# Ladme/groan_rs

Hardware: AMD Instinct MI355X
Metric: frames/sec RMSD-fit, 1e6 atoms triclinic, 1/2/4/8 GPUs; HBM GB/s vs peak (higher is better)
Workload: dtype f32 (fp64 accumulators)

## Files before the change

### groan_rs_amd/csrc/gr_api.hip

```cpp
#include <hip/hip_runtime.h>

#include <cmath>
#include <cstdio>
#include <cstdlib>
#include <cstring>
#include <map>
#include <string>
#include <vector>

#include "../../include/groan_hip.h"
#include "gr_batch.h"
#include "gr_container.h"
#include "gr_kernels.h"
#include "gr_hot.h"
#include "gr_resident.h"
#include "gr_small.h"
#include "gr_xtc.h"
#include "gr_shape.h"
#include "gr_xtc_dev.h"
#include "gr_xtc_enc_dev.h"
#include "gr_trr.h"
#include "gr_cellgrid.h"
#include "gr_textio.h"
#include "gr_pool.h"
// ... 499 lines not shown
        if ((spins & 1023u) == 1023u && std::chrono::steady_clock::now() - t0 > std::chrono::milliseconds(20)) {
            c->small_sync_fallbacks++;
            HIPCHK(c, hipStreamSynchronize(c->stream));
            if (w[0] != seq || w[words - 1] != seq) return fail(c, GR_E_HIP, "a single-wave kernel ended without publishing its result");
            break;
        }
    }
    std::atomic_thread_fence(std::memory_order_acquire);
    c->small_calls++;
    return GR_OK;
}

static int res_next_epoch(gr_ctx *c, uint32_t *epoch) {
    if (++c->res_epoch == 0u) {
        HIPCHK(c, hipStreamSynchronize(c->stream));
        if (c->res_wgrec) HIPCHK(c, hipMemset(c->res_wgrec, 0, c->res_wgrec_cap * sizeof(unsigned long long)));
        HIPCHK(c, hipMemset(c->res_rec, 0, (size_t)GR_MAX_BATCH * 16 * sizeof(unsigned long long)));
        HIPCHK(c, hipMemset(c->res_abort + 2, 0, 2 * sizeof(uint32_t)));
        c->res_epoch = 1u;
    }
    *epoch = c->res_epoch;
    return GR_OK;
}
static int res_test_no_start(gr_ctx *c, uint32_t epoch) {
    if (!c->res_test_no_start) return GR_OK;
    const unsigned long long two = 2ull | ((unsigned long long)epoch << 32);
    c->res_test_no_start = 0;
    HIPCHK(c, hipMemcpyAsync(c->res_abort + 2, &two, sizeof two, hipMemcpyHostToDevice, c->stream));
    HIPCHK(c, hipStreamSynchronize(c->stream));
    return GR_OK;
}
template <int MODE>
static int res_close(gr_ctx *c, uint32_t nb, const double *fit_partials, uint32_t nparts, double sum_w, uint32_t epoch, bool fresh, uint32_t *seq) {
    const uint32_t sq = c->res_seq + 1u;
    k_res_close<MODE><<<dim3(nb), dim3(64), 0, c->stream>>>(fit_partials, nparts, sum_w, c->state_dev, c->res_rec, epoch, fresh ? 1u : 0u, c->res_abort, c->res_closed + nb,
                                                        c->res_out_dev->st, c->res_out_dev->words, &c->res_out_dev->seq, sq);
    HIPCHK(c, hipGetLastError());
    c->res_seq = sq; c->res_closed += nb; *seq = sq;
    return GR_OK;
}
static int res_collect(gr_ctx *c, uint32_t seq, uint32_t nb, uint32_t epoch, bool *started) {
    volatile uint32_t *w = &c->res_out->seq;
    const auto t0 = std::chrono::steady_clock::now();
    for (uint32_t spins = 0; *w != seq; ++spins) {
        if ((spins & 1023u) == 1023u && std::chrono::steady_clock::now() - t0 > std::chrono::milliseconds(20)) {
            c->res_sync_fallbacks++;
            HIPCHK(c, hipStreamSynchronize(c->stream));
            if (*w != seq) return fail(c, GR_E_HIP, "the kernel behind the resident pass ended without publishing its results");
            break;
        }
    }
    std::atomic_thread_fence(std::memory_order_acquire);
    memcpy(c->state_host, c->res_out->st, (size_t)nb * sizeof(GrFrameState));
    memcpy(c->res_words_host, c->res_out->words, 12 * sizeof(uint32_t));
    for (int k = 0; k < 2; ++k) { const uint32_t v = c->res_words_host[8 + k]; c->res_words_host[8 + k] = v - c->res_late_seen[k]; c->res_late_seen[k] = v; }
    *started = c->res_words_host[2] == 1u && c->res_words_host[3] == epoch;
    if (!*started || c->res_words_host[0]) HIPCHK(c, hipStreamSynchronize(c->stream));
    return GR_OK;
}

int center_stage(gr_ctx *c, uint32_t first_slot, uint32_t nf, const GrSel &sel, int kind, int weighted,
                 int mass_first, int target, int only_status = 0) {
    if (small_ok(c, sel)) {
        k_center_small_stage<<<dim3(nf), dim3(64), 0, c->stream>>>(c->frames, c->frame_stride, first_slot, c->masses, sel, c->boxes_dev, kind, weighted, mass_first, target, c->state_dev, only_status);
        HIPCHK(c, hipGetLastError());
        return GR_OK;
    }
    uint32_t nch = chunks_for(sel);
    if (nf > 1 && nch >= 8) nch &= ~7u;
    const dim3 grid(nch, nf), wg(GR_WG);
    if (kind == 0) k_center_sums<0><<<grid, wg, 0, c->stream>>>(c->frames, c->frame_stride, first_slot, c->masses, sel, c->boxes_dev, c->state_dev, weighted, c->cen_partials, only_status);
    else if (kind == 1) k_center_sums<1><<<grid, wg, 0, c->stream>>>(c->frames, c->frame_stride, first_slot, c->masses, sel, c->boxes_dev, c->state_dev, weighted, c->cen_partials, only_status);
    else k_center_sums<2><<<grid, wg, 0, c->stream>>>(c->frames, c->frame_stride, first_slot, c->masses, sel, c->boxes_dev, c->state_dev, weighted, c->cen_partials, only_status);
    k_center_finalize<<<dim3(nf), dim3(GR_WG), 0, c->stream>>>(c->cen_partials, nch, c->boxes_dev, first_slot, kind, weighted, mass_first, target, sel.n, c->state_dev, only_status);
    HIPCHK(c, hipGetLastError());
    return GR_OK;
}

int pbc_center_stages(gr_ctx *c, uint32_t first_slot, uint32_t nf, const GrSel &sel, int weighted, int only_status = 0) {
    if (small_ok(c, sel) && only_status == 0) {
        k_center_small_pbc<<<dim3(nf), dim3(64), 0, c->stream>>>(c->frames, c->frame_stride, first_slot, c->masses, sel, c->boxes_dev, weighted, c->state_dev);
        HIPCHK(c, hipGetLastError());
        return GR_OK;
    }
    int st = center_stage(c, first_slot, nf, sel, 1, 0, 0, 0, only_status);
    if (st != GR_OK) return st;
    return center_stage(c, first_slot, nf, sel, 2, weighted, 0, 1, only_status);
}

// ... 972 lines not shown

static int states_from_prechecks(gr_ctx *c, const grb::PreView &pre) {
    if (pre.all_ok) return state_reset(c, pre.n);
    for (uint32_t f = 0; f < pre.n; ++f) { GrFrameState z = {}; z.err_index = GR_NOIDX; z.status = pre.pre[f]; c->state_host[f] = z; }
    HIPCHK(c, hipMemcpyAsync(c->state_dev, c->state_host, pre.n * sizeof(GrFrameState), hipMemcpyHostToDevice, c->stream));
    return GR_OK;
}
int gr_group_center_batch(gr_ctx *c, uint32_t first_slot, uint32_t n_frames, const char *group, int kind, int weighted, float *out, int *status_out) try {
    int st = slot_check(c, first_slot, n_frames); if (st) return st;
    (void)hipSetDevice(c->device);
    const Group *g = need_group(c, group, st, true); if (!g) return st;
    if (kind != GR_CENTER_NAIVE && kind != GR_CENTER_ESTIMATE && kind != GR_CENTER_PBC) return fail(c, GR_E_INVALID_ARG, "unknown centre kind");
    const GrSel sel = make_sel(*g);
    grb::FirstError<gr_ctx> fe;
    for (const auto [b0, nb, s0] : grb::Segments{ first_slot, n_frames }) {
        const grb::Prechecks pre(c, { b0, nb, s0 }, box_checks(c, kind != GR_CENTER_NAIVE));
        SlotUse use(c, s0, nb);
        st = states_from_prechecks(c, pre); if (st) return st;
        if (kind == GR_CENTER_NAIVE) st = center_stage(c, s0, nb, sel, 0, weighted, 0, 1);
        else if (kind == GR_CENTER_ESTIMATE) st = center_stage(c, s0, nb, sel, 1, weighted, 1, 1);
        else st = center_onepass_ok(c, sel) ? pbc_center_onepass(c, s0, nb, sel, weighted) : pbc_center_stages(c, s0, nb, sel, weighted);
        if (st) return st;
        st = fetch_states(c, nb); if (st) return st;
        std::vector<GrFrameState> res;
        st = center_redo_fallbacks(c, s0, nb, sel, weighted, res); if (st) return st;
        for (uint32_t f = 0; f < nb; ++f) {
            const int s = grb::close_frame(c, fe, pre, f, status_out, [&] { return frame_status(c, res[f]); });
            if (out) for (int k = 0; k < 3; ++k) out[3 * (size_t)(b0 + f) + k] = (s == GR_OK) ? res[f].com[k] : NAN;
        }
    }
    return fe.finish(c);
} catch (...) { return gr_abi_guard(); }
static int center_resident(gr_ctx *c, uint32_t s0, uint32_t nb, const GrSel &all, const GrSel &csel, int dim_mask, int weighted,
                           const std::vector<int> &pre, bool fresh_states, std::vector<uint8_t> &done, std::vector<uint8_t> &torn, bool &ran) {
    done.assign(nb, 0); torn.assign(nb, 0); ran = false;
    if (!c->center_resident || !csel.contiguous || csel.masked || !all.contiguous || all.start != 0 || all.n != c->n) return GR_OK;
    {
        bool ortho = true;
        for (uint32_t f = 0; f < nb; ++f) if (pre[f] == GR_OK) { ortho = c->boxes_host[s0 + f].ortho != 0; break; }
        if (c->resident == 1 && (uint64_t)csel.n * 100 < c->n * (ortho ? 15u : 3u)) return GR_OK;
    }
    if (small_ok(c, csel)) return GR_OK;
    uint32_t streams = 1, gwg = GR_RES_GROUPS;
    const uint32_t wgs = resident_wgs(c, true, nb, all, &streams, &gwg);
    if (!wgs) return GR_OK;
    if (!resident_acquire(c->device)) return GR_OK;
    struct Release { gr_ctx *c; ~Release() { resident_release(c->device); } } release{ c };
    hipStream_t S = c->stream;
    const uint32_t res_stream = wgs * streams;
    const uint32_t n_fin = std::min<uint32_t>(streams > 8 ? GR_RES_MAX_FIN : 8, c->res_max_wgs - res_stream);
    const size_t rec_words = (size_t)nb * ((wgs + GR_RES_REC_PAD - 1u) & ~(uint32_t)(GR_RES_REC_PAD - 1u)) * GR_RES_REC_WORDS;
    if (rec_words > c->res_wgrec_cap) {
        if (c->res_wgrec) (void)hipFree(c->res_wgrec);
        c->res_wgrec = nullptr; c->res_wgrec_cap = 0;
        HIPCHK(c, hipMalloc(&c->res_wgrec, rec_words * sizeof(unsigned long long)));
        HIPCHK(c, hipMemsetAsync(c->res_wgrec, 0, rec_words * sizeof(unsigned long long), S));
        c->res_wgrec_cap = rec_words;
    }
    GrResCtl ctl;
    memset(&ctl, 0, sizeof ctl);
    { const int se = res_next_epoch(c, &ctl.epoch); if (se) return se; }
    ctl.wgrec = c->res_wgrec; ctl.rec = c->res_rec; ctl.abort = c->res_abort; ctl.progress = c->res_progress; ctl.n_stream = res_stream; ctl.n_fin = n_fin;
    ctl.checkin_target = c->res_checkin + res_stream + n_fin; ctl.fresh_states = fresh_states ? 1u : 0u;
    ctl.wgs_frame = wgs; ctl.streams = streams; ctl.groups_wg = gwg;
    ctl.team_waves = resident_team_waves(wgs, streams);
    ctl.patience_ticks = (unsigned long long)c->wall_khz * 3000ull; ctl.start_ticks = (unsigned long long)c->wall_khz * 200ull;
    ctl.test_abort_frame = c->res_test_abort_at; c->res_test_abort_at = 0xFFFFFFFFu;
    ctl.metro_t16 = c->res_metro_ns >= 100 ? (uint32_t)std::min<uint64_t>(0xFFFFFFFFull, (uint64_t)c->res_metro_ns * (uint64_t)c->wall_khz * 16ull / 1000000ull) : 0u;
    ctl.metro_lead = (uint32_t)((uint64_t)c->wall_khz * 2000ull / 1000000ull);
    ctl.cen_weighted = weighted ? 1u : 0u; ctl.cen_dim_mask = (uint32_t)dim_mask;
    float *frames = c->frames; size_t stride = c->frame_stride; uint32_t slot0 = s0, nfr = nb, natoms = (uint32_t)c->n;
    const float *masses = c->masses; GrSel sel_arg = csel; const GrBox *boxes = c->boxes_dev; GrPlanDev plan; memset(&plan, 0, sizeof plan);
    GrFrameState *states = c->state_dev; double *fparts = nullptr;
    void *args[] = { &frames, &stride, &slot0, &nfr, &natoms, &masses, &sel_arg, &boxes, &plan, &states, &fparts, &ctl };
    bool ubox = true;
    for (uint32_t f = 1; f < nb && ubox; ++f) ubox = memcmp(&c->boxes_host[s0 + f], &c->boxes_host[s0], sizeof(GrBox)) == 0;
    const bool fit_last = c->res_fit_last ? c->res_fit_last == 2 : (uint64_t)res_stream * 10u >= (uint64_t)c->res_max_wgs * 9u;
    { const int sn = res_test_no_start(c, ctl.epoch); if (sn) return sn; }
    if (hipLaunchKernel(resident_center_fn(ubox, fit_last), dim3(res_stream + n_fin), dim3(GrResShape::LANES), args, GrResShape::LDS_BYTES, S) != hipSuccess) {
        (void)hipGetLastError();
        c->res_max_wgs = 0;
        return GR_OK;
    }
    c->res_checkin += res_stream + n_fin;
    uint32_t seq = 0; bool started = false;
    { const int sc = res_close<1>(c, nb, nullptr, 0u, 1.0, ctl.epoch, fresh_states, &seq); if (sc) return sc; }
    { const int sc = res_collect(c, seq, nb, ctl.epoch, &started); if (sc) return sc; }
    c->res_last_streams = streams;
    if (!started) {
        c->res_handshake_misses++;
        c->res_backoff = c->res_backoff ? std::min<uint32_t>(c->res_backoff * 2u, 1024u) : 4u;
        c->res_skip = c->res_backoff;
        return GR_OK;
    }
    c->res_backoff = 0;
    c->cen_res_launches++;
    if (fresh_states) c->res_lean_segments++;
    ran = true;
#ifdef GR_EXP_STEPTIME
    if (getenv("GR_STEPTIME")) {
        unsigned long long st[32];
        if (hipMemcpy(st, c->res_abort + 16, sizeof st, hipMemcpyDeviceToHost) == hipSuccess) {
            const double turns_ = (double)((nb + streams - 1) / streams + GrResShape::K);
            const char *who[4] = { "wg 0 wave 0", "wg 0 wave 5", "wg mid wave 0", "wg mid wave 5" };
            for (int w = 0; w < 4; ++w) {
                fprintf(stderr, "center steptime %-14s ticks/turn:", who[w]);
                double tot = 0; for (int k = 0; k < 7; ++k) tot += (double)st[w * 8 + k];
                const char *nm[7] = { "gate", "request", "rows+sums", "reduce+handover", "record wait", "fit+stores", "park" };
                for (int k = 0; k < 7; ++k) fprintf(stderr, " %s %.0f", nm[k], (double)st[w * 8 + k] / turns_);
// ... 39 lines not shown
        k_translate_wrap_rows<<<dim3(tiles * 3u, nb), dim3(64), 0, c->stream>>>(c->frames + (size_t)s0 * c->frame_stride, c->frame_stride, sel, c->boxes_dev + s0, c->state_dev, mode, dim_mask,
                                                                            v ? v[0] : 0.f, v ? v[1] : 0.f, v ? v[2] : 0.f, c->bad_dev);
        HIPCHK(c, hipGetLastError());
    } else if (g->n) {
        const uint64_t units = sel.contiguous ? ((uint64_t)sel.n + 3) / 4 + 128 : (sel.masked & 2u) ? ((uint64_t)sel.span + 3) / 4 + 128 : sel.n;
        const uint32_t nwg = (uint32_t)std::min<uint64_t>((units + GR_WG - 1) / GR_WG, 4096);
        k_translate_wrap<<<dim3(nwg, nb), dim3(GR_WG), stream_lds(c, GR_STREAM_WGS_CU_DEFAULT), c->stream>>>(c->frames + (size_t)s0 * c->frame_stride, c->frame_stride, sel, c->boxes_dev + s0, c->state_dev, mode, dim_mask,
                                                                       v ? v[0] : 0.f, v ? v[1] : 0.f, v ? v[2] : 0.f, c->bad_dev);
        HIPCHK(c, hipGetLastError());
    }
    HIPCHK(c, hipMemcpyAsync(c->bad_host, c->bad_dev, 4 * (size_t)nb * sizeof(uint32_t), hipMemcpyDeviceToHost, c->stream));
    HIPCHK(c, hipMemcpyAsync(c->state_host, c->state_dev, nb * sizeof(GrFrameState), hipMemcpyDeviceToHost, c->stream));
    HIPCHK(c, hipStreamSynchronize(c->stream));
    for (uint32_t f = 0; f < nb; ++f)
        grb::close_frame(c, fe, pre, f, status_out, [&]() -> int {
            if (mode == 1 && c->state_host[f].status != GR_OK) return frame_status(c, c->state_host[f]);
            return c->bad_host[4 * f] != GR_NOIDX ? fail(c, GR_E_NO_POSITION, "atom has no position", c->bad_host[4 * f]) : (int)GR_OK;
        });
    return GR_OK;
}
static int translate_batch_api(gr_ctx *c, uint32_t first_slot, uint32_t n_frames, const char *group, const float *v, const char *center_group, int dim, int weighted, int *status_out) {
    int st = slot_check(c, first_slot, n_frames); if (st) return st;
    (void)hipSetDevice(c->device);
    const Group *g = find_group(c, group ? group : "all");
    if (!g) return fail(c, GR_E_GROUP_NOT_FOUND, group);
    const Group *cg = nullptr;
    if (center_group) {
        cg = need_group(c, center_group, st, true); if (!cg) return st;
        if (dim < 0 || dim > 7) return fail(c, GR_E_INVALID_ARG, "bad dimension");
    }
    static const int mask[8] = { 0, 1, 2, 4, 3, 5, 6, 7 };
    grb::FirstError<gr_ctx> fe;
    for (const auto [b0, nb, s0] : grb::Segments{ first_slot, n_frames }) {
        const grb::Prechecks pre(c, { b0, nb, s0 }, box_checks(c, true));
        SlotUse use(c, s0, nb);
        const bool states_unset = cg != nullptr && pre.all_ok;
        if (!states_unset) { st = states_from_prechecks(c, pre); if (st) return st; }
        std::vector<uint8_t> done(nb, 0), torn(nb, 0);
        bool ran = false;
        if (cg) { st = center_resident(c, s0, nb, make_sel(*g), make_sel(*cg), mask[dim], weighted, pre.codes, states_unset, done, torn, ran); if (st) return st; }
        bool any_done = false;
        for (uint32_t f = 0; f < nb; ++f) any_done = any_done || done[f];
        if (any_done) {
            for (uint32_t f = 0; f < nb; ++f) {
                if (!done[f]) continue;
                grb::close_frame(c, fe, pre, f, status_out, [&]() -> int {
                    if (torn[f]) return fail(c, GR_E_HIP, "the resident atoms_center pass stalled while this frame was being moved: some of its atoms carry the new coordinates, others the original ones (frame index in gr_last_error_index)", pre.b0 + f);
                    return frame_status(c, c->state_host[f]);
                });
            }
            for (uint32_t a = 0; a < nb; ) {
                if (done[a]) { ++a; continue; }
                uint32_t b = a;
                while (b < nb && !done[b]) ++b;
                const grb::PreView run = pre.sub(a, b);
                st = states_from_prechecks(c, run); if (st) return st;
                st = center_stage(c, s0 + a, b - a, make_sel(*cg), 1, weighted, 1, 0); if (st) return st;
                st = translate_batch(c, run, g, v, 1, mask[dim], status_out, fe); if (st) return st;
                a = b;
            }
            continue;
        }
        if (ran || states_unset) { st = states_from_prechecks(c, pre); if (st) return st; }
        if (cg) { st = center_stage(c, s0, nb, make_sel(*cg), 1, weighted, 1, 0); if (st) return st; }
        st = translate_batch(c, pre, g, v, cg ? 1 : 2, cg ? mask[dim] : 7, status_out, fe); if (st) return st;
    }
    return fe.finish(c);
}
int gr_group_translate_batch(gr_ctx *c, uint32_t first_slot, uint32_t n_frames, const char *group, const float v[3], int *status_out) try {
    if (!c) return GR_E_INVALID_ARG;
    if (!v) return fail(c, GR_E_INVALID_ARG, "vector is NULL");
    return translate_batch_api(c, first_slot, n_frames, group, v, nullptr, 7, 0, status_out);
} catch (...) { return gr_abi_guard(); }
// ... 125 lines not shown
    case GR_TUNE_RESIDENT_FIT_LAST: if (value < 0 || value > 2) break; c->res_fit_last = (int)value; return GR_OK;
    case GR_TUNE_STREAM_WGS_PER_CU: if (value < 0 || value > 8) break; c->stream_wgs_cu = (int)value; return GR_OK;
    case GR_TUNE_CENTER_RESIDENT: if (value < 0 || value > 1) break; c->center_resident = (int)value; return GR_OK;
    case GR_TUNE_TRANSLATE_ROWS: if (value < 0 || value > 1) break; c->translate_rows = (int)value; return GR_OK;
    case GR_TUNE_RESIDENT_FILL: if (value < 1 || value > 16) break; c->res_fill16 = (int)value; return GR_OK;
    case GR_TUNE_RESIDENT_GROUPS: if (value != 2) break; return GR_OK;
    case GR_TUNE_TEST_RESIDENT_NO_START: c->res_test_no_start = value ? 1 : 0; return GR_OK;
    case GR_TUNE_TEST_RESIDENT_ABORT_AT: c->res_test_abort_at = value < 0 ? 0xFFFFFFFFu : (uint32_t)value; return GR_OK;
    default: break;
    }
    return fail(c, GR_E_INVALID_ARG, "unknown tuning key or value out of range");
} catch (...) { return gr_abi_guard(); }

static int rmsd_exact(gr_rmsd_plan *p, gr_ctx *c, const GrSel &sel, uint32_t first_slot, uint32_t nf, int fit) {
    int st = pbc_center_stages(c, first_slot, nf, sel, 1); if (st) return st;
    if (small_ok(c, sel)) {
        k_rmsd_small<1><<<dim3(nf), dim3(64), 0, c->stream>>>(c->frames, c->frame_stride, first_slot, c->masses, sel, c->boxes_dev, p->dev, c->state_dev, 1, nullptr, nullptr, 0u);
    } else {
        const uint32_t nch = chunks_for(sel);
        k_rmsd_accum<1><<<dim3(nch, nf), dim3(GR_WG), 0, c->stream>>>(c->frames, c->frame_stride, first_slot, c->masses, sel, c->boxes_dev, p->dev, c->state_dev, c->acc_partials);
        k_rmsd_finalize<1><<<dim3(nf), dim3(GR_WG), 0, c->stream>>>(c->acc_partials, nch, c->frames, c->frame_stride, first_slot, sel, c->boxes_dev, p->dev, c->state_dev);
    }
    if (fit) {
        const uint32_t gx = (uint32_t)std::min<uint64_t>(((c->n >> 2) + GR_WG * 4 - 1) / (GR_WG * 4) + 1, 1024);
        k_fit_pk<false><<<dim3(gx, nf), dim3(GR_WG), 0, c->stream>>>(c->frames, c->frame_stride, first_slot, (uint32_t)c->n, c->boxes_dev, p->dev, c->state_dev, c->masses, sel, nullptr);
    }
    HIPCHK(c, hipGetLastError());
    return GR_OK;
}

static int segment_begin(gr_rmsd_plan *p, uint32_t s0, uint32_t nb, int fit) {
    gr_ctx *c = p->target;
    Pending &q = p->pend;
    q = Pending();
    q.s0 = s0; q.nb = nb; q.fit = fit; q.active = true;
    SlotUse use(c, s0, nb);
    const Group *g = find_group(c, p->group.c_str());
    q.pre.assign(nb, GR_OK); q.pre_idx.assign(nb, 0); q.pre_msg.assign(nb, std::string());
    for (uint32_t f = 0; f < nb; ++f) {
        int s = box_check(c, s0 + f);
        if (s == GR_OK && !g) s = fail(c, GR_E_GROUP_NOT_FOUND, p->group);
        if (s == GR_OK && g->n == 0) s = fail(c, GR_E_EMPTY_GROUP, p->group);
        q.pre[f] = s;
        if (s != GR_OK) { q.pre_msg[f] = c->err; q.pre_idx[f] = c->err_index; }
        q.any_ok = q.any_ok || s == GR_OK;
    }
    if (!q.any_ok) return GR_OK;
    const GrSel sel = make_sel(*g);
    q.sel = sel; q.group_n = g->n; q.has_group = true;
    if (!p->resolved || p->resolved_epoch != c->epoch) {
        p->resolved_epoch = c->epoch;
        bool same = (g->n == p->n_ref);
        if (same) { size_t k = 0; for (uint64_t i : grc::expand(g->blocks)) { const float a = c->masses_host[i], b = p->w_host[k++]; if (!(a == b)) { same = false; break; } } }
        p->dev.w_is_mass = same ? 1u : 0u; p->resolved = true;
        p->span_ok = p->p_span_dev != nullptr && g->masked && g->mask_dev != nullptr && g->blocks == p->ref_blocks;
    }
    q.consistent = (g->n == p->n_ref);
    const bool fast_asked = c->two_pass && c->rmsd_fast && p->dev.w_is_mass != 0 && g->n >= c->rmsd_fast_min && ((!fit && sel.contiguous) || (sel.masked && p->span_ok));
    const bool small = q.consistent && !p->exact && small_ok(c, sel) && !fast_asked;
    if (small && nb == 1) {
        q.small = true; q.small_seq = ++c->small_seq;
        k_rmsd_small<0><<<dim3(1), dim3(64), 0, c->stream>>>(c->frames, c->frame_stride, s0, c->masses, sel, c->boxes_dev, p->dev,
                                                         c->state_dev, 0, c->small_state_dev, c->small_flag_dev, q.small_seq);
        if (fit) k_fit_pk<false><<<dim3(fit_grid(c, 1), 1), dim3(GR_WG), 0, c->stream>>>(c->frames, c->frame_stride, s0, (uint32_t)c->n, c->boxes_dev, p->dev, c->state_dev, c->masses, sel, nullptr);
        p->fit_behind_small = fit != 0;
        HIPCHK(c, hipGetLastError());
        return GR_OK;
    }
    bool states_unset = false;
    {
        bool all_ok = true;
        for (uint32_t f = 0; f < nb; ++f) all_ok = all_ok && q.pre[f] == GR_OK;
        states_unset = all_ok;
        if (!all_ok) {
            for (uint32_t f = 0; f < nb; ++f) { GrFrameState z = {}; z.err_index = GR_NOIDX; z.status = q.pre[f]; c->state_host[f] = z; }
            HIPCHK(c, hipMemcpyAsync(c->state_dev, c->state_host, nb * sizeof(GrFrameState), hipMemcpyHostToDevice, c->stream));
        }
    }
    auto zero_states = [&]() -> int { if (!states_unset) return GR_OK; states_unset = false; return state_reset(c, nb); };
    int st;
    if (!(q.consistent && !p->exact && !small)) { st = zero_states(); if (st) return st; }
    if (small) {
        k_rmsd_small<0><<<dim3(nb), dim3(64), 0, c->stream>>>(c->frames, c->frame_stride, s0, c->masses, sel, c->boxes_dev, p->dev, c->state_dev, 1, nullptr, nullptr, 0u);
        if (fit) k_fit_pk<false><<<dim3(fit_grid(c, nb), nb), dim3(GR_WG), 0, c->stream>>>(c->frames, c->frame_stride, s0, (uint32_t)c->n, c->boxes_dev, p->dev, c->state_dev, c->masses, sel, nullptr);
        HIPCHK(c, hipGetLastError());
    } else if (!q.consistent) {
        st = pbc_center_stages(c, s0, nb, sel, 1); if (st) return st;
    } else if (p->exact) {
        st = rmsd_exact(p, c, sel, s0, nb, fit); if (st) return st;
    } else {
        const uint32_t sb = c->sub_batch;
        const bool lite = fit && sel.contiguous && c->two_pass;
        const bool msk = sel.masked && p->span_ok;
        const bool fast = c->two_pass && c->rmsd_fast && p->dev.w_is_mass != 0 && g->n >= c->rmsd_fast_min && ((!fit && sel.contiguous) || msk);
        q.rmsd_fast = fast;
        p->dev.fast_sigmas = (float)c->rmsd_fast_sigmas;
        GrPlanDev plan_span = p->dev; plan_span.p = p->p_span_dev;
        const uint32_t n_groups = (nb + sb - 1) / sb;
        if (lite) {
            size_t need = 0;
            for (uint32_t f0 = 0; f0 < nb; f0 += sb) need = std::max(need, (size_t)nb * fit_grid(c, std::min<uint32_t>(sb, nb - f0)) * (GR_WG / 64));
            if (need > c->fit_partials_cap) {
                if (c->fit_partials) (void)hipFree(c->fit_partials);
                c->fit_partials = nullptr; c->fit_partials_cap = 0;
                HIPCHK(c, hipMalloc(&c->fit_partials, need * sizeof(double)));
// ... 40 lines not shown
                if (c->res_metro_ns >= 100) period_ns = (uint32_t)c->res_metro_ns;
                else if (c->res_metro_ns == 0) {
                    gr_ctx::Metro &m = c->metro;
                    if (m.shape != shape) { m = gr_ctx::Metro(); m.shape = shape; }
                    if (m.off_for) m.off_for--;
                    else if (m.free_ns > 0) period_ns = (uint32_t)(m.T_ns + 0.5);
                    q.res_metro_auto = true;
                }
                q.res_metro_ns = period_ns;
                ctl.metro_t16 = (uint32_t)std::min<uint64_t>(0xFFFFFFFFull, (uint64_t)period_ns * (uint64_t)c->wall_khz * 16ull / 1000000ull);
                ctl.metro_lead = (uint32_t)((uint64_t)c->wall_khz * 2000ull / 1000000ull);
            }
#ifdef GR_EXP_STEPTIME
            {
                static unsigned long long *dbg_dev = nullptr;
                if (!dbg_dev) (void)hipMalloc(&dbg_dev, (size_t)GR_MAX_CHUNKS * 8 * 4 * sizeof(unsigned long long));
                ctl.dbg = getenv("GR_STEPTIME") ? dbg_dev : nullptr;
                g_steptime_dbg = ctl.dbg;
            }
#endif
#ifdef GR_EXP_TIMELINE
            {
                static unsigned long long *tl_dev = nullptr; static size_t tl_cap = 0;
                if (nb > tl_cap) { if (tl_dev) (void)hipFree(tl_dev); tl_dev = nullptr; tl_cap = 0; if (hipMalloc(&tl_dev, (size_t)nb * 8 * sizeof(unsigned long long)) == hipSuccess) tl_cap = nb; }
                ctl.tl = getenv("GR_TIMELINE") ? tl_dev : nullptr;
                if (ctl.tl) HIPCHK(c, hipMemsetAsync(ctl.tl, 0, (size_t)nb * 8 * sizeof(unsigned long long), S));
                q.tl_dev = ctl.tl;
            }
#endif
            float *frames = c->frames; size_t stride = c->frame_stride; uint32_t slot0 = s0, nfr = nb, natoms = (uint32_t)c->n;
            const float *masses = c->masses; GrSel sel_arg = sel; const GrBox *boxes = c->boxes_dev; GrPlanDev plan = res_msk ? plan_span : p->dev;
            GrFrameState *states = c->state_dev; double *fparts = c->fit_partials;
            void *args[] = { &frames, &stride, &slot0, &nfr, &natoms, &masses, &sel_arg, &boxes, &plan, &states, &fparts, &ctl };
            bool ubox = true;
            for (uint32_t f = 1; f < nb && ubox; ++f) ubox = memcmp(&c->boxes_host[s0 + f], &c->boxes_host[s0], sizeof(GrBox)) == 0;
#ifdef GR_EXP_NO_UBOX
            ubox = false;
#endif
            const bool whole = sel.start == 0 && sel.n == c->n;
            const bool fit_last = c->res_fit_last ? c->res_fit_last == 2 : (uint64_t)res_stream * 10u >= (uint64_t)c->res_max_wgs * 9u;
            const void *fn = resident_fn(p->dev.w_is_mass != 0, ubox, whole, fit_last);
            const uint32_t lanes = GrResShape::LANES, lds = GrResShape::LDS_BYTES;
            st = res_test_no_start(c, ctl.epoch); if (st) return st;
            if (c->profile) EVREC(c, c->pev[0], true, S);
            const hipError_t le = hipLaunchKernel(fn, dim3(res_stream + n_fin), dim3(lanes), args, lds, S);
            if (le == hipSuccess) {
                if (c->profile) EVREC(c, c->pev[1], true, S);
                c->res_checkin += res_stream + n_fin;
                q.res_fresh = states_unset; q.res_epoch = ctl.epoch;
                states_unset = false;
                st = res_close<0>(c, nb, c->fit_partials, res_wgs * GrResShape::WAVES, p->dev.sw, ctl.epoch, q.res_fresh, &q.res_seq); if (st) return st;
                q.resident = true; q.res_stream = res_stream; q.res_streams = res_streams;
                q.rmsd_fast = false;
                c->res_last_streams = res_streams;
            } else {
                (void)hipGetLastError();
                c->res_max_wgs = 0;
                resident_done(c);
            }
        }
        if (!q.resident) { st = zero_states(); if (st) return st; }
        for (uint32_t g = 0; g < n_groups && !q.resident; ++g) {
            const uint32_t f0 = g * sb, nf = std::min<uint32_t>(sb, nb - f0), nch = batch_chunks(c, sel, nf), gx = fit_grid(c, nf);
            GrAccPartial *parts = c->acc_partials + (size_t)f0 * GR_MAX_CHUNKS;
            if (c->profile) EVREC(c, c->pev[6 * g], true, S);
            if (lite) k_sums_pk<false><<<dim3(nch, nf), dim3(GR_WG), 0, S>>>(c->frames, c->frame_stride, s0 + f0, c->masses, sel, c->boxes_dev, p->dev, parts,
                                                                             fused ? c->fuse_cnt + f0 : nullptr, c->state_dev + f0);
            else if (fast && msk) k_sums_pk<false, true, true><<<dim3(nch, nf), dim3(GR_WG), 0, S>>>(c->frames, c->frame_stride, s0 + f0, c->masses, sel, c->boxes_dev, plan_span, parts,
// ... 15 lines not shown
                else k_fit_pk<false><<<dim3(gx, nf), dim3(GR_WG), 0, S>>>(c->frames, c->frame_stride, s0 + f0, (uint32_t)c->n, c->boxes_dev, p->dev, c->state_dev + f0, c->masses, sel, nullptr);
                if (c->profile) EVREC(c, c->pev[6 * g + 5], true, S);
                if (lite) k_rmsd_close<<<dim3(nf), dim3(64), 0, S>>>(c->fit_partials + (size_t)f0 * gx * (GR_WG / 64), gx * (GR_WG / 64), p->dev.sw, c->state_dev + f0);
            }
        }
        HIPCHK(c, hipGetLastError());
        if (c->profile) q.n_prof_groups = q.resident ? 0 : n_groups;
    }
    if (!q.resident) HIPCHK(c, hipMemcpyAsync(c->state_host, c->state_dev, nb * sizeof(GrFrameState), hipMemcpyDeviceToHost, c->stream));
    return GR_OK;
}

static int segment_end(gr_rmsd_plan *p, float *rmsd_out, int *status_out, float *R_out, std::vector<GrFrameState> *final_states = nullptr) {
    gr_ctx *c = p->target;
    Pending &q = p->pend;
    if (!q.active) return fail(c, GR_E_INVALID_ARG, "no batch in flight");
    q.active = false;
    const uint32_t nb = q.nb, s0 = q.s0;
    const int fit = q.fit;
    grb::FirstError<gr_ctx> fe;
    if (!q.any_ok) {
        for (uint32_t f = 0; f < nb; ++f) {
            c->err = q.pre_msg[f]; c->err_index = q.pre_idx[f]; fe.note(c, q.pre[f]);
            if (status_out) status_out[f] = q.pre[f];
            if (rmsd_out) rmsd_out[f] = NAN;
            if (R_out) for (int k = 0; k < 9; ++k) R_out[9 * (size_t)f + k] = NAN;
        }
        if (final_states) { final_states->assign(nb, GrFrameState{}); for (uint32_t f = 0; f < nb; ++f) { (*final_states)[f].status = q.pre[f]; (*final_states)[f].err_index = GR_NOIDX; } }
    } else {
        if (!q.has_group) return fail(c, GR_E_INVALID_ARG, "batch state lost");
        const GrSel sel = q.sel;
        bool res_started = false;
        if (q.small) { const int sw = small_wait(c, q.small_seq); if (sw) return sw; c->state_host[0] = *c->small_state; }
        else if (q.resident) { const int sw = res_collect(c, q.res_seq, nb, q.res_epoch, &res_started); if (sw) { resident_done(c); return sw; } }
        else HIPCHK(c, hipStreamSynchronize(c->stream));
        std::vector<uint8_t> redo;
        std::vector<uint8_t> torn;
#ifdef GR_EXP_TIMELINE
        if (q.resident && q.tl_dev) {
            std::vector<unsigned long long> tl((size_t)nb * 8);
            if (hipMemcpy(tl.data(), q.tl_dev, tl.size() * sizeof(unsigned long long), hipMemcpyDeviceToHost) == hipSuccess) {
                double sum[8] = { 0 }; double period = 0; uint64_t n = 0, polled = 0, fpolls = 0; unsigned long long prev = 0;
                for (uint32_t f = 0; f < nb; ++f) {
                    const unsigned long long *t = &tl[(size_t)f * 8];
                    if (!t[0] || !t[1] || !t[5] || !(t[6] & 0xFFFFFFFFFFFFull)) continue;
                    const unsigned long long look = t[6] & 0xFFFFFFFFFFFFull;
                    sum[0] += (double)((long long)(t[1] - t[0])); sum[1] += (double)((long long)(t[2] - t[1])); sum[2] += (double)((long long)(t[3] - t[2]));
                    sum[3] += (double)((long long)(t[4] - t[3])); sum[4] += (double)((long long)(t[5] - t[4])); sum[5] += (double)((long long)(look - t[5]));
                    sum[6] += (double)((long long)(look - t[0]));
                    if (prev) period += (double)((long long)(t[0] - prev));
                    prev = t[0];
                    polled += (t[6] >> 48) != 0; fpolls += t[7]; n++;
                }
                if (n > 1) fprintf(stderr, "timeline (%llu frames, us): pub->all records %.2f | ->team totals %.2f | state load %.2f | closing %.2f | publish+store %.2f | ->wg0 looks %.2f | pub->look %.2f | period %.3f | wg0 polled for %.0f %% of the frames | finalizer polls per frame %.1f\n",
                                   (unsigned long long)n, sum[0] / n / 100.0, sum[1] / n / 100.0, sum[2] / n / 100.0, sum[3] / n / 100.0, sum[4] / n / 100.0, sum[5] / n / 100.0, sum[6] / n / 100.0,
                                   period / (n - 1) / 100.0, 100.0 * polled / n, (double)fpolls / n);
            }
        }
#endif
        if (q.resident) {
            resident_done(c);
            if (!res_started) {
                c->res_handshake_misses++;
                c->res_backoff = c->res_backoff ? std::min<uint32_t>(c->res_backoff * 2u, 1024u) : 4u;
                c->res_skip = c->res_backoff + 1u;
                const int fit_again = q.fit;
                const uint32_t s0_again = q.s0, nb_again = q.nb;
                int st2 = segment_begin(p, s0_again, nb_again, fit_again);
// ... 97 lines not shown
                        const double next = T * 0.985;
                        if (m.fail_ns == 0 || next > m.fail_ns * 1.004) m.T_ns = next;
                        else if (m.best_ns > m.free_ns * 0.98) {
                            m.off_for = 512; m.free_ns = 0; m.T_ns = 0; m.best_ns = 0; m.fail_ns = 0;
                        }
                        else if (++m.held >= 64) { m.held = 0; m.fail_ns *= 0.995; }
                    } else {
                        m.fail_ns = std::max(m.fail_ns, T);
                        m.T_ns = m.best_ns > T ? m.best_ns : T * 1.02;
                        if (m.best_ns > 0 && m.best_ns <= T) m.best_ns = 0;
                        if (m.T_ns >= m.free_ns * 0.995) {
                            m.off_for = 512; m.free_ns = 0; m.T_ns = 0; m.best_ns = 0; m.fail_ns = 0;
                        }
                    }
                }
            }
            if (c->profile) {
                float ms = 0.f;
                hipError_t ee = hipEventElapsedTime(&ms, c->pev[0], c->pev[1]);
                if (ee == hipErrorNotReady) { (void)hipGetLastError(); HIPCHK(c, hipEventSynchronize(c->pev[1])); ee = hipEventElapsedTime(&ms, c->pev[0], c->pev[1]); }
                HIPCHK(c, ee);
                c->prof_ms[3] += ms; c->prof_launches[3] += 1; c->prof_frames[3] += nb;
            }
        }
        for (uint32_t gi = 0; gi < q.n_prof_groups; ++gi) {
            const uint32_t nf = std::min<uint32_t>(c->sub_batch, nb - gi * c->sub_batch);
            for (int k = 0; k < 3; ++k) {
                if ((k == 1 && q.fused) || (k == 2 && !fit)) continue;
                float ms = 0.f;
                HIPCHK(c, hipEventElapsedTime(&ms, c->pev[6 * gi + 2 * k], c->pev[6 * gi + 2 * k + 1]));
                c->prof_ms[k] += ms; c->prof_launches[k] += 1; c->prof_frames[k] += nf;
            }
        }
        std::vector<GrFrameState> res(c->state_host, c->state_host + nb);
        if (!redo.empty()) {
            const int keep = c->resident;
            c->resident = 0;
            int st_redo = GR_OK;
            for (uint32_t f0 = 0; f0 < nb && st_redo == GR_OK; ) {
                if (!redo[f0]) { ++f0; continue; }
                uint32_t f1 = f0;
                while (f1 < nb && redo[f1]) ++f1;
                std::vector<GrFrameState> fs2;
                Pending sub;
                std::swap(sub, p->pend);
                st_redo = segment_begin(p, s0 + f0, f1 - f0, fit);
                if (st_redo == GR_OK) {
                    const int st_nested = segment_end(p, nullptr, nullptr, nullptr, &fs2);
                    if (fs2.size() != (size_t)(f1 - f0)) st_redo = st_nested != GR_OK ? st_nested : GR_E_HIP;
                    else for (uint32_t f = f0; f < f1; ++f) res[f] = fs2[f - f0];
                } else { p->pend.active = false; resident_done(c); }
                std::swap(sub, p->pend);
                c->res_redone_frames += f1 - f0;
                f0 = f1;
            }
            c->resident = keep;
            if (st_redo != GR_OK) return st_redo;
        }
        if (q.rmsd_fast) {
            for (uint32_t f0 = 0; f0 < nb; ) {
                if (res[f0].status != GR_ST_REDO_EXACT) { if (q.pre[f0] == GR_OK) c->rmsd_fast_frames++; ++f0; continue; }
                uint32_t f1 = f0;
                while (f1 < nb && res[f1].status == GR_ST_REDO_EXACT) ++f1;
                const uint32_t nf = f1 - f0, nch = batch_chunks(c, sel, nf);
                SlotUse use(c, s0 + f0, nf);
                int st = state_reset(c, nf); if (st) return st;
// ... 1051 lines not shown
```

### groan_rs_amd/csrc/gr_resident.h

```cpp
#pragma once
#include <type_traits>
#include "gr_hot.h"

struct GrResShape {
    static constexpr int LANES = 512, WAVES = LANES / 64;
#ifndef GR_RES_K
#define GR_RES_K 6
#endif
    static constexpr int K = GR_RES_K;
    static constexpr int R = 8;
    static constexpr int PARK_F4 = K * 3 * LANES;
    static constexpr int WSUM_F = R * WAVES * 32;
#ifdef GR_EXP_TIMELINE
    static constexpr int TL_BYTES = 128 * 4 * 8;
#else
    static constexpr int TL_BYTES = 0;
#endif
    static constexpr int LDS_BYTES = PARK_F4 * 16 + WSUM_F * 4 + R * WAVES * 8 + 3 * R * 4 + 2 * WAVES * 4 + TL_BYTES;
    static constexpr int REC_PER_WAVE = 256 / WAVES, LANES_PER_REC = 64 / REC_PER_WAVE, WORDS_PER_LANE = 32 / LANES_PER_REC;
};
#ifndef GR_RES_SLEEP
#define GR_RES_SLEEP 2
#endif
#ifndef GR_RES_BAL
// ... 912 lines not shown
        ctl.progress[wg_all * WAVES + wave] = n_fitted;
        (void)__hip_atomic_fetch_max(reinterpret_cast<unsigned long long *>(ctl.abort + 6), (unsigned long long)wall_clock64(), __ATOMIC_RELAXED, __HIP_MEMORY_SCOPE_AGENT);
        if (n_late) (void)__hip_atomic_fetch_add(ctl.abort + 8, n_late, __ATOMIC_RELAXED, __HIP_MEMORY_SCOPE_AGENT);
        if (n_waited) (void)__hip_atomic_fetch_add(ctl.abort + 9, n_waited, __ATOMIC_RELAXED, __HIP_MEMORY_SCOPE_AGENT);
#ifdef GR_EXP_STEPTIME
        if (ctl.dbg) {
            unsigned long long *o = ctl.dbg + (size_t)(wg_all * WAVES + wave) * 4u;
            unsigned long long tot = 0; for (int k = 0; k < 7; ++k) tot += st_acc[k];
            o[0] = st_acc[4]; o[1] = st_acc[7] | (st_combines << 32);
            o[2] = (__builtin_amdgcn_s_getreg((20 << 0) | (0 << 6) | (3 << 11)) & 7u) | (simd_of[wave] << 8);
            o[3] = tot;
        }
        if ((wg_all == 0u || wg_all == ctl.n_stream / 2u) && (wave == 0u || wave == 5u)) {
            unsigned long long *o = reinterpret_cast<unsigned long long *>(ctl.abort + 16) + ((wg_all ? 2u : 0u) + (wave ? 1u : 0u)) * 8u;
            for (int k = 0; k < 8; ++k) o[k] = st_acc[k];
        }
#endif
        if (clk_wave) {
            const unsigned long long dc = (unsigned long long)clock64() - clk_c0, dw = (unsigned long long)wall_clock64() - clk_w0;
            gr_st_agent(ctl.abort + 10, (uint32_t)(dc >> 8)); gr_st_agent(ctl.abort + 11, (uint32_t)(dw >> 8));
        }
    }
#ifdef GR_EXP_TIMELINE
    if (tl_wg && wave == 0 && !bail) {
        for (uint32_t t = (n_turns > 128u ? n_turns - 128u : 0u) + lane; t < n_turns; t += 64u) {
            const size_t f = kf(t);
            ctl.tl[f * 8 + 0] = tls[(t & 127u) * 4u + 0u];
            ctl.tl[f * 8 + 6] = tls[(t & 127u) * 4u + 1u] | (tls[(t & 127u) * 4u + 2u] << 48);
        }
    }
#endif
}

template <int MODE>
__global__ __launch_bounds__(64) void k_res_close(const double *__restrict__ fit_partials, uint32_t nparts, double sum_w, GrFrameState *state,
                                                  const unsigned long long *__restrict__ rec, uint32_t epoch, uint32_t fresh_states, uint32_t *ctl_words,
                                                  uint32_t done_target, GrFrameState *out_states, uint32_t *out_words, uint32_t *out_seq, uint32_t seq) {
    constexpr uint32_t NW = sizeof(GrFrameState) / 4u, W_RMSD = offsetof(GrFrameState, rmsd) / 4u, W_STATUS = offsetof(GrFrameState, status) / 4u;
    static_assert(sizeof(GrFrameState) % 4u == 0 && NW <= 64u, "a frame state is exported by one wave, a word per lane");
    const uint32_t frame = blockIdx.x, lane = threadIdx.x;
    uint32_t *sw = reinterpret_cast<uint32_t *>(state + frame);
    uint32_t w = 0u;
    if (fresh_states && (uint32_t)(gr_ld_agent(rec + (size_t)frame * 16u) >> 32) != epoch) {
        GrFrameState z = {};
        z.err_index = GR_NOIDX; z.status = GR_ST_ABORTED;
        if (lane < NW) { w = reinterpret_cast<const uint32_t *>(&z)[lane]; sw[lane] = w; }
    } else if (lane < NW) w = sw[lane];
    const int status = __shfl((int)w, (int)W_STATUS, 64);
    if (MODE == 0 && status == 0) {
        double s0 = 0.0, s1 = 0.0, s2 = 0.0, s3 = 0.0;
        const double *p = fit_partials + (size_t)frame * nparts;
        uint32_t k = lane;
        for (; k + 192 < nparts; k += 256) { s0 += p[k]; s1 += p[k + 64]; s2 += p[k + 128]; s3 += p[k + 192]; }
        for (; k < nparts; k += 64) s0 += p[k];
        const double s = gr_wave_sum((s0 + s1) + (s2 + s3));
        float r = 0.0f;
        if (lane == 0) { r = (float)sqrt(fmax(s, 0.0) / sum_w); state[frame].rmsd = r; }
        r = __shfl(r, 0, 64);
        if (lane == W_RMSD) w = __float_as_uint(r);
    }
    if (lane < NW) reinterpret_cast<uint32_t *>(out_states + frame)[lane] = w;
    __threadfence_system();
    uint32_t n = 0u;
    if (lane == 0) n = __hip_atomic_fetch_add(ctl_words + 12, 1u, __ATOMIC_ACQ_REL, __HIP_MEMORY_SCOPE_AGENT) + 1u;
    n = (uint32_t)__builtin_amdgcn_readfirstlane((int)n);
    if (n != done_target) return;
    if (lane < 12u) out_words[lane] = gr_ld_agent(ctl_words + lane);
    __threadfence_system();
    if (lane == 0) __hip_atomic_store(out_seq, seq, __ATOMIC_RELEASE, __HIP_MEMORY_SCOPE_SYSTEM);
}
```

Measured before the change: 142,300.

## Batch close kernel frames per workgroup and skip host state copies on fast path

The close kernel now handles several frames per workgroup: it stages each frame's state in LDS and writes to host-mapped output with 16-byte stores, which cuts the number of system-scope fences and atomic check-ins. On the fast path with all frames OK, the host reads results straight from mapped memory and skips the full state memcpy and vector copy. Box-uniformity checks are folded into the precheck loops, and precheck vectors reuse their allocations. This adds more complex control flow and a new dependence on mapped-memory reads.

```diff
diff --git a/groan_rs_amd/csrc/gr_api.hip b/groan_rs_amd/csrc/gr_api.hip
--- a/groan_rs_amd/csrc/gr_api.hip
+++ b/groan_rs_amd/csrc/gr_api.hip
@@ -555,14 +555,14 @@
 }
 template <int MODE>
 static int res_close(gr_ctx *c, uint32_t nb, const double *fit_partials, uint32_t nparts, double sum_w, uint32_t epoch, bool fresh, uint32_t *seq) {
-    const uint32_t sq = c->res_seq + 1u;
-    k_res_close<MODE><<<dim3(nb), dim3(64), 0, c->stream>>>(fit_partials, nparts, sum_w, c->state_dev, c->res_rec, epoch, fresh ? 1u : 0u, c->res_abort, c->res_closed + nb,
-                                                        c->res_out_dev->st, c->res_out_dev->words, &c->res_out_dev->seq, sq);
+    const uint32_t sq = c->res_seq + 1u, wgs = (nb + GR_RES_CLOSE_W - 1u) / GR_RES_CLOSE_W;
+    k_res_close<MODE><<<dim3(wgs), dim3(64 * GR_RES_CLOSE_W), 0, c->stream>>>(fit_partials, nparts, sum_w, c->state_dev, nb, c->res_rec, epoch, fresh ? 1u : 0u, c->res_abort, c->res_closed + wgs,
+                                                                          c->res_out_dev->st, c->res_out_dev->words, &c->res_out_dev->seq, sq);
     HIPCHK(c, hipGetLastError());
-    c->res_seq = sq; c->res_closed += nb; *seq = sq;
-    return GR_OK;
-}
-static int res_collect(gr_ctx *c, uint32_t seq, uint32_t nb, uint32_t epoch, bool *started) {
+    c->res_seq = sq; c->res_closed += wgs; *seq = sq;
+    return GR_OK;
+}
+static int res_collect(gr_ctx *c, uint32_t seq, uint32_t nb, uint32_t epoch, bool *started, bool copy_states = true) {
     volatile uint32_t *w = &c->res_out->seq;
     const auto t0 = std::chrono::steady_clock::now();
     for (uint32_t spins = 0; *w != seq; ++spins) {
@@ -574,10 +574,10 @@
         }
     }
     std::atomic_thread_fence(std::memory_order_acquire);
-    memcpy(c->state_host, c->res_out->st, (size_t)nb * sizeof(GrFrameState));
     memcpy(c->res_words_host, c->res_out->words, 12 * sizeof(uint32_t));
     for (int k = 0; k < 2; ++k) { const uint32_t v = c->res_words_host[8 + k]; c->res_words_host[8 + k] = v - c->res_late_seen[k]; c->res_late_seen[k] = v; }
     *started = c->res_words_host[2] == 1u && c->res_words_host[3] == epoch;
+    if (copy_states || !*started || c->res_words_host[0]) memcpy(c->state_host, c->res_out->st, (size_t)nb * sizeof(GrFrameState));
     if (!*started || c->res_words_host[0]) HIPCHK(c, hipStreamSynchronize(c->stream));
     return GR_OK;
 }
@@ -1616,7 +1616,7 @@
     return fe.finish(c);
 } catch (...) { return gr_abi_guard(); }
 static int center_resident(gr_ctx *c, uint32_t s0, uint32_t nb, const GrSel &all, const GrSel &csel, int dim_mask, int weighted,
-                           const std::vector<int> &pre, bool fresh_states, std::vector<uint8_t> &done, std::vector<uint8_t> &torn, bool &ran) {
+                           const std::vector<int> &pre, bool fresh_states, bool ubox, std::vector<uint8_t> &done, std::vector<uint8_t> &torn, bool &ran) {
     done.assign(nb, 0); torn.assign(nb, 0); ran = false;
     if (!c->center_resident || !csel.contiguous || csel.masked || !all.contiguous || all.start != 0 || all.n != c->n) return GR_OK;
     {
@@ -1657,8 +1657,6 @@
     const float *masses = c->masses; GrSel sel_arg = csel; const GrBox *boxes = c->boxes_dev; GrPlanDev plan; memset(&plan, 0, sizeof plan);
     GrFrameState *states = c->state_dev; double *fparts = nullptr;
     void *args[] = { &frames, &stride, &slot0, &nfr, &natoms, &masses, &sel_arg, &boxes, &plan, &states, &fparts, &ctl };
-    bool ubox = true;
-    for (uint32_t f = 1; f < nb && ubox; ++f) ubox = memcmp(&c->boxes_host[s0 + f], &c->boxes_host[s0], sizeof(GrBox)) == 0;
     const bool fit_last = c->res_fit_last ? c->res_fit_last == 2 : (uint64_t)res_stream * 10u >= (uint64_t)c->res_max_wgs * 9u;
     { const int sn = res_test_no_start(c, ctl.epoch); if (sn) return sn; }
     if (hipLaunchKernel(resident_center_fn(ubox, fit_last), dim3(res_stream + n_fin), dim3(GrResShape::LANES), args, GrResShape::LDS_BYTES, S) != hipSuccess) {
@@ -1764,13 +1762,18 @@
     static const int mask[8] = { 0, 1, 2, 4, 3, 5, 6, 7 };
     grb::FirstError<gr_ctx> fe;
     for (const auto [b0, nb, s0] : grb::Segments{ first_slot, n_frames }) {
-        const grb::Prechecks pre(c, { b0, nb, s0 }, box_checks(c, true));
+        bool ubox = true;
+        const uint32_t seg_s0 = s0;
+        const grb::Prechecks pre(c, { b0, nb, s0 }, [&](uint32_t slot) {
+            if (cg && ubox && slot != seg_s0) ubox = memcmp(&c->boxes_host[slot], &c->boxes_host[seg_s0], sizeof(GrBox)) == 0;
+            return box_check(c, slot);
+        });
         SlotUse use(c, s0, nb);
         const bool states_unset = cg != nullptr && pre.all_ok;
         if (!states_unset) { st = states_from_prechecks(c, pre); if (st) return st; }
         std::vector<uint8_t> done(nb, 0), torn(nb, 0);
         bool ran = false;
-        if (cg) { st = center_resident(c, s0, nb, make_sel(*g), make_sel(*cg), mask[dim], weighted, pre.codes, states_unset, done, torn, ran); if (st) return st; }
+        if (cg) { st = center_resident(c, s0, nb, make_sel(*g), make_sel(*cg), mask[dim], weighted, pre.codes, states_unset, ubox, done, torn, ran); if (st) return st; }
         bool any_done = false;
         for (uint32_t f = 0; f < nb; ++f) any_done = any_done || done[f];
         if (any_done) {
@@ -1962,18 +1965,26 @@
 static int segment_begin(gr_rmsd_plan *p, uint32_t s0, uint32_t nb, int fit) {
     gr_ctx *c = p->target;
     Pending &q = p->pend;
-    q = Pending();
+    {
+        std::vector<int> pre = std::move(q.pre); std::vector<uint64_t> pre_idx = std::move(q.pre_idx); std::vector<std::string> pre_msg = std::move(q.pre_msg);
+        q = Pending();
+        q.pre = std::move(pre); q.pre_idx = std::move(pre_idx); q.pre_msg = std::move(pre_msg);
+    }
     q.s0 = s0; q.nb = nb; q.fit = fit; q.active = true;
     SlotUse use(c, s0, nb);
     const Group *g = find_group(c, p->group.c_str());
-    q.pre.assign(nb, GR_OK); q.pre_idx.assign(nb, 0); q.pre_msg.assign(nb, std::string());
+    q.pre.assign(nb, GR_OK); q.pre_idx.clear(); q.pre_msg.clear();
+    bool all_ok = true, ubox_all = true;
     for (uint32_t f = 0; f < nb; ++f) {
         int s = box_check(c, s0 + f);
         if (s == GR_OK && !g) s = fail(c, GR_E_GROUP_NOT_FOUND, p->group);
         if (s == GR_OK && g->n == 0) s = fail(c, GR_E_EMPTY_GROUP, p->group);
-        q.pre[f] = s;
-        if (s != GR_OK) { q.pre_msg[f] = c->err; q.pre_idx[f] = c->err_index; }
-        q.any_ok = q.any_ok || s == GR_OK;
+        if (s != GR_OK) {
+            if (q.pre_msg.empty()) { q.pre_msg.resize(nb); q.pre_idx.assign(nb, 0); }
+            q.pre[f] = s; q.pre_msg[f] = c->err; q.pre_idx[f] = c->err_index;
+            all_ok = false;
+        } else q.any_ok = true;
+        if (f && ubox_all) ubox_all = memcmp(&c->boxes_host[s0 + f], &c->boxes_host[s0], sizeof(GrBox)) == 0;
     }
     if (!q.any_ok) return GR_OK;
     const GrSel sel = make_sel(*g);
@@ -1999,8 +2010,6 @@
     }
     bool states_unset = false;
     {
-        bool all_ok = true;
-        for (uint32_t f = 0; f < nb; ++f) all_ok = all_ok && q.pre[f] == GR_OK;
         states_unset = all_ok;
         if (!all_ok) {
             for (uint32_t f = 0; f < nb; ++f) { GrFrameState z = {}; z.err_index = GR_NOIDX; z.status = q.pre[f]; c->state_host[f] = z; }
@@ -2107,8 +2116,7 @@
             const float *masses = c->masses; GrSel sel_arg = sel; const GrBox *boxes = c->boxes_dev; GrPlanDev plan = res_msk ? plan_span : p->dev;
             GrFrameState *states = c->state_dev; double *fparts = c->fit_partials;
             void *args[] = { &frames, &stride, &slot0, &nfr, &natoms, &masses, &sel_arg, &boxes, &plan, &states, &fparts, &ctl };
-            bool ubox = true;
-            for (uint32_t f = 1; f < nb && ubox; ++f) ubox = memcmp(&c->boxes_host[s0 + f], &c->boxes_host[s0], sizeof(GrBox)) == 0;
+            bool ubox = ubox_all;
 #ifdef GR_EXP_NO_UBOX
             ubox = false;
 #endif
@@ -2190,8 +2198,9 @@
         const GrSel sel = q.sel;
         bool res_started = false;
         if (q.small) { const int sw = small_wait(c, q.small_seq); if (sw) return sw; c->state_host[0] = *c->small_state; }
-        else if (q.resident) { const int sw = res_collect(c, q.res_seq, nb, q.res_epoch, &res_started); if (sw) { resident_done(c); return sw; } }
+        else if (q.resident) { const int sw = res_collect(c, q.res_seq, nb, q.res_epoch, &res_started, !(q.res_fresh && !final_states)); if (sw) { resident_done(c); return sw; } }
         else HIPCHK(c, hipStreamSynchronize(c->stream));
+        const bool states_mapped = q.resident && q.res_fresh && !final_states && res_started && !c->res_words_host[0];
         std::vector<uint8_t> redo;
         std::vector<uint8_t> torn;
 #ifdef GR_EXP_TIMELINE
@@ -2355,6 +2364,20 @@
                 c->prof_ms[k] += ms; c->prof_launches[k] += 1; c->prof_frames[k] += nf;
             }
         }
+        if (states_mapped) {
+            const GrFrameState *ms = c->res_out->st;
+            bool all_closed = true;
+            for (uint32_t f = 0; f < nb && all_closed; ++f) all_closed = ms[f].status == GR_OK;
+            if (all_closed) {
+                for (uint32_t f = 0; f < nb; ++f) {
+                    if (status_out) status_out[f] = GR_OK;
+                    if (rmsd_out) rmsd_out[f] = ms[f].rmsd;
+                    if (R_out) for (int k = 0; k < 9; ++k) R_out[9 * (size_t)f + k] = ms[f].R[k];
+                }
+                return GR_OK;
+            }
+            memcpy(c->state_host, ms, (size_t)nb * sizeof(GrFrameState));
+        }
         std::vector<GrFrameState> res(c->state_host, c->state_host + nb);
         if (!redo.empty()) {
             const int keep = c->resident;
diff --git a/groan_rs_amd/csrc/gr_resident.h b/groan_rs_amd/csrc/gr_resident.h
--- a/groan_rs_amd/csrc/gr_resident.h
+++ b/groan_rs_amd/csrc/gr_resident.h
@@ -968,34 +968,48 @@
 #endif
 }
 
+#ifndef GR_RES_CLOSE_W
+#define GR_RES_CLOSE_W 8
+#endif
 template <int MODE>
-__global__ __launch_bounds__(64) void k_res_close(const double *__restrict__ fit_partials, uint32_t nparts, double sum_w, GrFrameState *state,
+__global__ __launch_bounds__(64 * GR_RES_CLOSE_W) void k_res_close(const double *__restrict__ fit_partials, uint32_t nparts, double sum_w, GrFrameState *state, uint32_t nframes,
                                                   const unsigned long long *__restrict__ rec, uint32_t epoch, uint32_t fresh_states, uint32_t *ctl_words,
                                                   uint32_t done_target, GrFrameState *out_states, uint32_t *out_words, uint32_t *out_seq, uint32_t seq) {
-    constexpr uint32_t NW = sizeof(GrFrameState) / 4u, W_RMSD = offsetof(GrFrameState, rmsd) / 4u, W_STATUS = offsetof(GrFrameState, status) / 4u;
-    static_assert(sizeof(GrFrameState) % 4u == 0 && NW <= 64u, "a frame state is exported by one wave, a word per lane");
-    const uint32_t frame = blockIdx.x, lane = threadIdx.x;
-    uint32_t *sw = reinterpret_cast<uint32_t *>(state + frame);
-    uint32_t w = 0u;
-    if (fresh_states && (uint32_t)(gr_ld_agent(rec + (size_t)frame * 16u) >> 32) != epoch) {
-        GrFrameState z = {};
-        z.err_index = GR_NOIDX; z.status = GR_ST_ABORTED;
-        if (lane < NW) { w = reinterpret_cast<const uint32_t *>(&z)[lane]; sw[lane] = w; }
-    } else if (lane < NW) w = sw[lane];
-    const int status = __shfl((int)w, (int)W_STATUS, 64);
-    if (MODE == 0 && status == 0) {
-        double s0 = 0.0, s1 = 0.0, s2 = 0.0, s3 = 0.0;
-        const double *p = fit_partials + (size_t)frame * nparts;
-        uint32_t k = lane;
-        for (; k + 192 < nparts; k += 256) { s0 += p[k]; s1 += p[k + 64]; s2 += p[k + 128]; s3 += p[k + 192]; }
-        for (; k < nparts; k += 64) s0 += p[k];
-        const double s = gr_wave_sum((s0 + s1) + (s2 + s3));
-        float r = 0.0f;
-        if (lane == 0) { r = (float)sqrt(fmax(s, 0.0) / sum_w); state[frame].rmsd = r; }
-        r = __shfl(r, 0, 64);
-        if (lane == W_RMSD) w = __float_as_uint(r);
-    }
-    if (lane < NW) reinterpret_cast<uint32_t *>(out_states + frame)[lane] = w;
+    constexpr uint32_t W = GR_RES_CLOSE_W, NW = sizeof(GrFrameState) / 4u, W_RMSD = offsetof(GrFrameState, rmsd) / 4u, W_STATUS = offsetof(GrFrameState, status) / 4u, W_ERR = offsetof(GrFrameState, err_index) / 4u;
+    static_assert(sizeof(GrFrameState) % 4u == 0 && NW <= 64u, "a frame state goes to LDS a word per lane");
+    static_assert((W * sizeof(GrFrameState)) % 16u == 0, "a workgroup's frames begin on a 16-byte boundary of out_states");
+    __shared__ __attribute__((aligned(16))) uint32_t rows[W * NW];
+    const uint32_t lane = threadIdx.x & 63u, wave = threadIdx.x >> 6, frame0 = blockIdx.x * W, frame = frame0 + wave;
+    if (frame < nframes) {
+        uint32_t *sw = reinterpret_cast<uint32_t *>(state + frame);
+        uint32_t w = 0u;
+        if (fresh_states && (uint32_t)(gr_ld_agent(rec + (size_t)frame * 16u) >> 32) != epoch) {
+            w = lane == W_STATUS ? (uint32_t)GR_ST_ABORTED : lane == W_ERR ? (uint32_t)GR_NOIDX : 0u;
+            if (lane < NW) sw[lane] = w;
+        } else if (lane < NW) w = sw[lane];
+        const int status = __shfl((int)w, (int)W_STATUS, 64);
+        if (MODE == 0 && status == 0) {
+            double s0 = 0.0, s1 = 0.0, s2 = 0.0, s3 = 0.0;
+            const double *p = fit_partials + (size_t)frame * nparts;
+            uint32_t k = lane;
+            for (; k + 192 < nparts; k += 256) { s0 += p[k]; s1 += p[k + 64]; s2 += p[k + 128]; s3 += p[k + 192]; }
+            for (; k < nparts; k += 64) s0 += p[k];
+            const double s = gr_wave_sum((s0 + s1) + (s2 + s3));
+            float r = 0.0f;
+            if (lane == 0) { r = (float)sqrt(fmax(s, 0.0) / sum_w); state[frame].rmsd = r; }
+            r = __shfl(r, 0, 64);
+            if (lane == W_RMSD) w = __float_as_uint(r);
+        }
+        if (lane < NW) rows[wave * NW + lane] = w;
+    }
+    __syncthreads();
+    if (wave != 0u) return;
+    {
+        const uint32_t nf = nframes - frame0 < W ? nframes - frame0 : W, nwords = nf * NW, n4 = nwords >> 2;
+        uint32_t *dst = reinterpret_cast<uint32_t *>(out_states + frame0);
+        for (uint32_t i = lane; i < n4; i += 64u) reinterpret_cast<uint4 *>(dst)[i] = reinterpret_cast<const uint4 *>(rows)[i];
+        if (lane < (nwords & 3u)) dst[4u * n4 + lane] = rows[4u * n4 + lane];
+    }
     __threadfence_system();
     uint32_t n = 0u;
     if (lane == 0) n = __hip_atomic_fetch_add(ctl_words + 12, 1u, __ATOMIC_ACQ_REL, __HIP_MEMORY_SCOPE_AGENT) + 1u;
```

New measurement: 141,300. About the same (-0.7%).
